# treangenlab/Seqwin

Hardware: AMD Instinct MI355X
Metric: Gbp/s minimizer-indexed (higher is better)
Workload: dtype u64

## Files before the change

seqwin_amd/csrc/device.hpp:

```cpp
#pragma once

#include <hip/hip_runtime.h>

#include <functional>
#include <memory>
#include <string>

#include "common.hpp"

namespace sw {

#define SW_HIP(expr)                                                                                   \
    do {                                                                                               \
        hipError_t _e = (expr);                                                                        \
        if (_e != hipSuccess)                                                                          \
            ::sw::raise(SW_ERR_DEVICE, "HIP error %d (%s) at %s:%d: %s", (int)_e, hipGetErrorString(_e), \
                        __FILE__, __LINE__, #expr);                                                    \
    } while (0)

__host__ __device__ inline uint64_t mix64(uint64_t x)
{
    x ^= x >> 30; x *= 0xbf58476d1ce4e5b9ULL;
    x ^= x >> 27; x *= 0x94d049bb133111ebULL;
    x ^= x >> 31;
// ... 170 lines not shown
};

namespace sw {

struct MultiGraph {
    std::vector<std::unique_ptr<sw_index>> slices;
    std::vector<uint32_t> record_offsets;
    std::string ids_blob;
    uint64_t n_assemblies = 0, total_bp = 0;
    const char *hash_route = "";
    std::string copy_route;
};
std::vector<int> devices_from_env();
void build_multi_device(const char *const *paths, size_t n_paths, uint64_t k, uint64_t w, uint64_t n_cpu, std::vector<int> devs,
                        MultiGraph &out, uint64_t chunk_bp = 0);

Plan &get_plan(sw_batch &b, uint64_t k, uint64_t w, bool *cached = nullptr);

struct SketchOut {
    DevArray<uint64_t> stage_hash;
    DevArray<uint64_t> stage_kmer;
    DevArray<uint32_t> tile_count;
    DevArray<uint64_t> tile_offset;
    uint64_t n_occ = 0;
    uint64_t launches = 0;
    uint64_t n_ovf_tiles = 0;
};
void run_sketch(const sw_batch &b, const Plan &plan, hipStream_t stream, SketchOut &out, float *sketch_ms);

void radix_sort_keys64(uint64_t *&keys, uint64_t *&alt, uint64_t n, unsigned begin_bit, unsigned end_bit, hipStream_t stream,
                       uint32_t *d_fail, bool perm_hi32 = false, unsigned long long *d_hist_given = nullptr, unsigned layout_bits = 0);
void radix_layout(unsigned bits, unsigned *digit_bits, unsigned *n_passes);
bool radix_unsort_perm(uint64_t *&keys, uint64_t *&alt, uint64_t n, unsigned low_bits, unsigned nbit, hipStream_t stream, uint32_t *d_fail);

void sort_keys64(uint64_t *&keys, uint64_t *&keys_alt, size_t n, unsigned begin_bit, unsigned end_bit, hipStream_t stream,
                 uint32_t *d_fail, bool perm_hi32 = false, unsigned long long *d_hist_given = nullptr, unsigned layout_bits = 0);
bool sort_keys64_is_own(size_t n);
void check_sort_failed(uint32_t fail_word);

struct alignas(16) OccPay {
    uint32_t low, pos, rec, idx;
};
int radix_rank_mode();
bool radix_pairs_available();
uint64_t radix_trim_state();
void radix_demote_rank();
constexpr uint32_t STAGE_WIN = 32;
constexpr uint32_t STAGE_ROW = STAGE_WIN + 9;
constexpr uint32_t STAGE_PAD = 1;
struct StageSource {
    const uint64_t *stage_hash, *stage_kmer;
    const uint32_t *tile_count;
    const uint64_t *tile_offset;
    const uint64_t *dst_off;
    uint32_t n_tiles;
    uint64_t mult;
    uint32_t *rec_out;
    const unsigned long long *chunk_dir;
    const uint64_t *rows;
};
void radix_sort_pairs32(uint32_t *&keys, uint32_t *&keys_alt, OccPay *&vals, OccPay *&vals_alt, uint64_t n, unsigned end_bit,
                        hipStream_t stream, uint32_t *d_fail, const StageSource *src = nullptr,
                        const std::function<void()> &after_first = std::function<void()>(), uint32_t *low_out = nullptr);
bool sort_pairs32(uint32_t *&keys, uint32_t *&keys_alt, OccPay *&vals, OccPay *&vals_alt, uint64_t n, unsigned end_bit,
                  hipStream_t stream, uint32_t *d_fail, uint32_t *low_out = nullptr);
struct PartState;
// ... 79 lines not shown
```

seqwin_amd/csrc/index.hip:

```cpp
#include <cstdlib>
#include <cstring>
#include <map>
#include <memory>

#include <rocprim/rocprim.hpp>

#include "device.hpp"

namespace sw {

namespace {

constexpr int TPB = 256;
inline unsigned blocks_for(uint64_t n, int per = TPB) { return (unsigned)((n + per - 1) / per); }
inline bool ranks_by_table()
{
    const char *e = SW_TEST_GETENV("SEQWIN_AMD_RANKS");
    return e && !strcmp(e, "table");
}

template <class K, class V>
void sort_pairs(K *&keys, K *&keys_alt, V *&vals, V *&vals_alt, size_t n, unsigned begin_bit, unsigned end_bit,
                hipStream_t stream)
{
// ... 2814 lines not shown
        }
    }
    DevArray<uint64_t> ukeys(m);
    DevArray<uint32_t> usum(m);
    DevArray<uint32_t> ucount(1);
    {
        auto flags = rocprim::make_transform_iterator(rocprim::make_counting_iterator<uint64_t>(0), PackedChangeAny{keys});
        const PackedPairEq eq{pshift, pmask};
        size_t tmp_bytes = 0;
        SW_HIP(rocprim::reduce_by_key(nullptr, tmp_bytes, keys, flags, m, ukeys.p, usum.p, ucount.p, rocprim::plus<uint32_t>(), eq,
                                      stream));
        DevArray<unsigned char> tmp(tmp_bytes);
        SW_HIP(rocprim::reduce_by_key(tmp.p, tmp_bytes, keys, flags, m, ukeys.p, usum.p, ucount.p, rocprim::plus<uint32_t>(), eq,
                                      stream));
        hipLaunchKernelGGL(k_drop_sentinel_run, dim3(1), dim3(1), 0, stream, ukeys.p, sentinel, ucount.p);
        SW_HIP(hipGetLastError());
        uint32_t n_edges = 0, failed = 0;
        SW_HIP(hipMemcpyAsync(&n_edges, ucount.p, 4, hipMemcpyDeviceToHost, stream));
        SW_HIP(hipMemcpyAsync(&failed, sort_fail.p, 4, hipMemcpyDeviceToHost, stream));
        SW_HIP(hipStreamSynchronize(stream));
        check_sort_failed(failed);
        ix.n_edges = n_edges;
    }
    if (ix.n_edges == 0) return;
    ix.edges.alloc(ix.n_edges);
    hipLaunchKernelGGL(k_edges_runs<false>, dim3(blocks_for(ix.n_edges)), dim3(TPB), 0, stream, ukeys.p, usum.p, pshift, pmask,
                       (uint64_t)ix.n_edges, nb, ix.nodes.p, rank_hash, ix.edges.p);
    SW_HIP(hipGetLastError());
    SW_HIP(hipStreamSynchronize(stream));
}
}

namespace {
struct WideKeys {
    unsigned lo_bits, hi_bits;
    uint64_t lo_base;
    RankHash hash;
};
void edges_from_pairs(uint64_t *keys, uint64_t *keys_alt, uint64_t m, uint64_t sentinel, unsigned nb, unsigned ab,
                      uint64_t *ck, uint32_t *ca, const unsigned long long *d_n_cand, uint64_t host_n_cand,
                      const uint64_t *rank_hash, hipStream_t stream, sw_index &ix, hipEvent_t rank_hash_ready = nullptr,
                      unsigned long long *d_hist = nullptr, const WideKeys *wide = nullptr)
{
    ix.n_edges = 0;
    if (m == 0) return;
    const unsigned key_bits = wide ? wide->lo_bits + wide->hi_bits : 2 * nb;
    DevArray<uint32_t> sort_fail(1);
    SW_HIP(hipMemsetAsync(sort_fail.p, 0, 4, stream));
    unsigned low_bits = 0, skip = 0, digit_bits = 0, n_passes = 0;
    if (sort_keys64_is_own(m)) {
        radix_layout(key_bits, &digit_bits, &n_passes);
        const unsigned hb = wide ? wide->hi_bits : nb;
        skip = hb >= digit_bits + 8 ? 1 : 0;
        if (skip && hb >= 2 * digit_bits + 8 && ix.n_nodes && m <= 4 * ix.n_nodes) skip = 2;
        if (const char *e = SW_TEST_GETENV("SEQWIN_AMD_EDGE_SKIP_PASSES")) skip = (unsigned)atoi(e);
        skip = std::min(skip, n_passes - 1);
        low_bits = skip * digit_bits;
    }
    sort_keys64(keys, keys_alt, m, low_bits, key_bits, stream, sort_fail.p, false,
                d_hist ? d_hist + ((size_t)skip << digit_bits) : nullptr, key_bits);
    RepairState rep;
    if (low_bits) enqueue_repair(EdgeKeyView{keys, low_bits}, EdgeKeyView{keys, low_bits}, ~0ull, m, nullptr, 0, rep, stream);
    DevArray<uint64_t> ukeys(m);
    DevArray<uint32_t> ucnt(m + 1), ucount(2);
    unsigned long long n_cand = host_n_cand;
    const char *rle_env = SW_AB_GETENV("SEQWIN_AMD_RLE");
    const bool own_rle = !(rle_env && !strcmp(rle_env, "rocprim"));
    bool demoted = false;
    for (int attempt = 0;; ++attempt) {
        SW_HIP(hipMemsetAsync(ucount.p + 1, 0, 4, stream));
        if (own_rle) {
            const unsigned blocks = (unsigned)((m + RLE_TILE - 1) / RLE_TILE);
            DevArray<unsigned long long> tile_state(blocks);
            DevArray<uint32_t> ticket(1);
            SW_HIP(hipMemsetAsync(tile_state.p, 0, (size_t)blocks * 8, stream));
            SW_HIP(hipMemsetAsync(ticket.p, 0, 4, stream));
            hipLaunchKernelGGL(k_rle_keys, dim3(blocks), dim3(RLE_THREADS), 0, stream, (const uint64_t *)keys, m, ukeys.p, ucnt.p, tile_state.p,
                               ticket.p, ucount.p, ucount.p + 1);
            SW_HIP(hipGetLastError());
        } else {
#ifdef SW_AB
            hipLaunchKernelGGL(k_check_ascending, dim3(blocks_for(m)), dim3(TPB), 0, stream, (const uint64_t *)keys, m, ucount.p + 1);
            size_t tmp_bytes = 0;
            SW_HIP(rocprim::run_length_encode(nullptr, tmp_bytes, keys, m, ukeys.p, ucnt.p, ucount.p, stream));
            DevArray<unsigned char> tmp(tmp_bytes);
            SW_HIP(rocprim::run_length_encode(tmp.p, tmp_bytes, keys, m, ukeys.p, ucnt.p, ucount.p, stream));
            SW_HIP(hipStreamSynchronize(stream));
#endif
        }
        hipLaunchKernelGGL(k_drop_sentinel_run, dim3(1), dim3(1), 0, stream, ukeys.p, sentinel, ucount.p);
        SW_HIP(hipGetLastError());
        uint32_t n_edges = 0, failed = 0, left = 0, descents = 0;
        SW_HIP(hipMemcpyAsync(&n_edges, ucount.p, 4, hipMemcpyDeviceToHost, stream));
        SW_HIP(hipMemcpyAsync(&descents, ucount.p + 1, 4, hipMemcpyDeviceToHost, stream));
        SW_HIP(hipMemcpyAsync(&failed, sort_fail.p, 4, hipMemcpyDeviceToHost, stream));
        if (low_bits && attempt == 0) SW_HIP(hipMemcpyAsync(&left, rep.status.p, 4, hipMemcpyDeviceToHost, stream));
        if (d_n_cand) SW_HIP(hipMemcpyAsync(&n_cand, d_n_cand, 8, hipMemcpyDeviceToHost, stream));
        SW_HIP(hipStreamSynchronize(stream));
        check_sort_failed(failed);
        if (low_bits && attempt == 0 && getenv("SEQWIN_AMD_DEBUG_EDGE_REPAIR")) {
            unsigned long long nd[2] = {0, 0};
            uint32_t st[2] = {0, 0};
// ... 1125 lines not shown
```

seqwin_amd/csrc/radix.hip:

```cpp
#include <algorithm>
#include <cstdlib>
#include <cstring>
#include <vector>
#include <map>
#include <mutex>

#include "device.hpp"

namespace sw {
namespace {

constexpr int RS_ITEMS = 16;
#ifdef SW_RS_STAMPS
__device__ unsigned long long *g_rs_stamps = nullptr;
#define RS_STAMP(i)                                                                                        \
    do {                                                                                                   \
        if (g_rs_stamps && (tile & 63u) == 0 && threadIdx.x == 0) g_rs_stamps[(size_t)(tile >> 6) * 16 + (i)] = clock64(); \
    } while (0)
#else
#define RS_STAMP(i) do { } while (0)
#endif
#ifndef RS_LOOK
#define RS_LOOK 4
#endif
// ... 33 lines not shown
{
    constexpr uint32_t RADIX = 1u << BITS;
    const unsigned p = blockIdx.x, at = begin_bit + BITS * p, sh = at - 32u, bits = min((unsigned)BITS, end_bit - at);
    const uint64_t v = threadIdx.x, block = 1ull << sh, period = block << bits;
    unsigned long long c = 0;
    if (v < (1ull << bits)) {
        const uint64_t q = n / period, r = n % period, lo = v * block;
        c = q * block + (r > lo ? (r - lo < block ? r - lo : block) : 0ull);
    }
    hist[(size_t)p * RADIX + threadIdx.x] = c;
}

constexpr uint32_t RS_CURSOR_STRIDE = 32;
template <int BITS> __global__ void k_rs_scan(unsigned long long *__restrict__ h, unsigned long long *__restrict__ cursor)
{
    constexpr uint32_t RADIX = 1u << BITS;
    __shared__ unsigned long long s[RADIX];
    const unsigned long long v = h[threadIdx.x];
    s[threadIdx.x] = v;
    __syncthreads();
    for (uint32_t d = 1; d < RADIX; d <<= 1) {
        const unsigned long long add = threadIdx.x >= d ? s[threadIdx.x - d] : 0;
        __syncthreads();
        s[threadIdx.x] += add;
        __syncthreads();
    }
    h[threadIdx.x] = s[threadIdx.x] - v;
    if (cursor) cursor[(size_t)threadIdx.x * RS_CURSOR_STRIDE] = s[threadIdx.x] - v;
}

#ifdef SW_AB
constexpr unsigned long long RS_AGG = 1ull << 62, RS_INC = 2ull << 62, RS_VAL = (1ull << 62) - 1ull;
#endif

template <int BITS>
__device__ __forceinline__ void match_digit(uint32_t d, bool live, uint32_t &mlo, uint32_t &mhi)
{
    const uint64_t lv = __ballot(live);
    mlo = (uint32_t)lv;
    mhi = (uint32_t)(lv >> 32);
#pragma unroll
    for (int b = 0; b < BITS; ++b) {
        const uint32_t sx = (uint32_t)(-(int32_t)((d >> b) & 1u));
        const uint64_t bal = __ballot(sx != 0);
        const uint32_t blo = (uint32_t)bal, bhi = (uint32_t)(bal >> 32);
        uint32_t nlo, nhi;
        asm("v_bitop3_b32 %0, %1, %2, %3 bitop3:0x90" : "=v"(nlo) : "v"(mlo), "s"(blo), "v"(sx));
        asm("v_bitop3_b32 %0, %1, %2, %3 bitop3:0x90" : "=v"(nhi) : "v"(mhi), "s"(bhi), "v"(sx));
        mlo = nlo;
        mhi = nhi;
    }
}

__global__ __launch_bounds__(1024) void k_rs_rank_selftest(uint32_t *__restrict__ mismatches)
{
    constexpr int BITS = 9;
    constexpr uint32_t RADIX = 1u << BITS, WAVES = 16;
    __shared__ uint16_t wa[WAVES][RADIX], wb[WAVES][RADIX];
    const uint32_t tid = threadIdx.x, lane = tid & 63u, wave = tid >> 6;
    for (uint32_t i = tid; i < WAVES * RADIX; i += 1024) (&wa[0][0])[i] = (&wb[0][0])[i] = 0;
    __syncthreads();
    uint32_t bad = 0;
    for (uint32_t r = 0; r < 96; ++r) {
        uint32_t x = (lane * 0x9E3779B1u) ^ ((r + 1u) * 0x85EBCA6Bu) ^ ((wave + blockIdx.x * 16u + 1u) * 0xC2B2AE35u);
        x ^= x >> 15; x *= 0x2C1B3C6Du; x ^= x >> 12;
        uint32_t d;
// ... 167 lines not shown
        goff[d] = digit_base[d] + excl - before;
    }
    __syncthreads();
#pragma unroll
    for (int i = 0; i < RS_ITEMS; ++i) {
        const uint32_t li = wave * (64 * RS_ITEMS) + i * 64 + lane;
        if (li < cnt_tile) {
            const uint32_t d = (uint32_t)(key[i] >> shift) & dmask;
            sk[lstart[d] + whist[wave][d] + rank[i]] = key[i];
        }
    }
    __syncthreads();
#pragma unroll
    for (int j = 0; j < RS_ITEMS; ++j) {
        const uint32_t t = j * THREADS + tid;
        if (t < cnt_tile) {
            const uint64_t k = sk[t];
            out[goff[(uint32_t)(k >> shift) & dmask] + t] = k;
        }
    }
}
#endif

constexpr unsigned long long RSE_VAL = (1ull << 46) - 1ull;
__device__ __forceinline__ unsigned long long rse_pack(uint32_t epoch, uint32_t flag, unsigned long long v)
{
    return ((unsigned long long)epoch << 48) | ((unsigned long long)flag << 46) | v;
}
__device__ __forceinline__ uint32_t rse_flag(unsigned long long w, uint32_t epoch)
{
    return (uint32_t)(w >> 48) == epoch ? (uint32_t)(w >> 46) & 3u : 0u;
}

template <int THREADS, int BITS, int RANK>
__global__ __launch_bounds__(THREADS) void k_rs_pass_p(const uint64_t *__restrict__ in, uint64_t *__restrict__ out, uint64_t n,
                                                       uint32_t n_tiles, unsigned shift, unsigned bits,
                                                       const unsigned long long *__restrict__ digit_base,
                                                       unsigned long long *__restrict__ state, uint32_t *__restrict__ ticket,
                                                       uint32_t *__restrict__ fail, uint32_t dbg,
                                                       unsigned long long *__restrict__ cursor, uint32_t cursor_stride,
                                                       uint32_t group_shift, uint32_t epoch)
{
    constexpr uint32_t RADIX = 1u << BITS, WAVES = THREADS / 64, TILE = THREADS * RS_ITEMS;
    static_assert(RADIX <= (uint32_t)THREADS, "one thread per digit");
    __shared__ uint64_t sk[TILE];
    __shared__ uint16_t whist[WAVES][RADIX];
    __shared__ uint32_t lstart[RADIX];
    __shared__ unsigned long long goff[RADIX];
    __shared__ uint32_t wsum[RADIX / 64];
    __shared__ uint32_t s_tile;
    const uint32_t tid = threadIdx.x, lane = tid & 63u, wave = tid >> 6;
    const uint32_t dmask = (1u << bits) - 1u;
    if (tid == 0) s_tile = atomicAdd(ticket, 1u);
    __syncthreads();
    uint32_t tile = s_tile;
    uint64_t key[RS_ITEMS];
    uint32_t rank[RS_ITEMS];
#pragma unroll
    for (int i = 0; i < RS_ITEMS; ++i) {
        const uint64_t g = (uint64_t)tile * TILE + wave * (64 * RS_ITEMS) + i * 64 + lane;
        key[i] = (tile < n_tiles && g < n) ? in[g] : ~0ull;
    }
    const uint32_t tid0 = threadIdx.x;
    uint32_t fut = 0;
    if (tid0 == 0) fut = atomicAdd(ticket, 1u);
    while (tile < n_tiles) {
        uint32_t tid = tid0;
        asm volatile("" : "+v"(tid));
        const uint32_t lane = tid & 63u, wave = tid >> 6;
        RS_STAMP(0);
        for (uint32_t i = tid; i < WAVES * RADIX / 2; i += THREADS) (reinterpret_cast<uint32_t *>(&whist[0][0]))[i] = 0;
        __syncthreads();
        const uint64_t t0 = (uint64_t)tile * TILE;
        const uint32_t cnt_tile = (uint32_t)min((uint64_t)TILE, n - t0);
        if constexpr (RANK == 1) {
#pragma unroll
            for (int i = 0; i < RS_ITEMS; ++i) {
                const uint32_t li = wave * (64 * RS_ITEMS) + i * 64 + lane;
                const uint32_t d = (uint32_t)(key[i] >> shift) & dmask;
                rank[i] = 0;
                if (li < cnt_tile) rank[i] = atomicAdd(reinterpret_cast<uint32_t *>(&whist[wave][d & ~1u]), 1u << ((d & 1u) << 4));
            }
#pragma unroll
            for (int i = 0; i < RS_ITEMS; ++i) {
                const uint32_t d = (uint32_t)(key[i] >> shift) & dmask;
                rank[i] = (rank[i] >> ((d & 1u) << 4)) & 0xFFFFu;
            }
            if ((dbg & 16u) && !cursor && wave == 0) {
#pragma unroll
                for (int i = 0; i < RS_ITEMS; ++i) {
                    const uint32_t li = i * 64 + lane;
                    const uint32_t d = li < cnt_tile ? ((uint32_t)(key[i] >> shift) & dmask) : ~lane;
                    const uint32_t od = __shfl_xor(d, 1, 64), orank = __shfl_xor(rank[i], 1, 64);
                    if (od == d) rank[i] = orank;
                }
            }
        }
#pragma unroll
        for (int i = 0; i < RS_ITEMS; ++i) {
            const uint32_t li = wave * (64 * RS_ITEMS) + i * 64 + lane;
            const bool live = li < cnt_tile;
            const uint32_t d = (uint32_t)(key[i] >> shift) & dmask;
            if constexpr (RANK == 1) {
                (void)live;
                (void)d;
            } else {
                uint32_t mlo = 1u << (lane & 31u), mhi = 0;
                if (!(dbg & 8u)) match_digit<BITS>(d, live, mlo, mhi);
                const uint32_t below = __builtin_amdgcn_mbcnt_hi(mhi, __builtin_amdgcn_mbcnt_lo(mlo, 0u));
                uint32_t prior = 0;
                if (live) prior = whist[wave][d];
                rank[i] = prior + below;
                __builtin_amdgcn_wave_barrier();
                if (live && below == 0) whist[wave][d] = (uint16_t)(prior + (uint32_t)__popc(mlo) + (uint32_t)__popc(mhi));
                __builtin_amdgcn_wave_barrier();
            }
        }
        RS_STAMP(1);
        __syncthreads();
        RS_STAMP(2);
        uint32_t total = 0, incl = 0;
        unsigned long long pre[RS_LOOK];
        unsigned long long *st = state + (size_t)tile * RADIX;
        if (tid < RADIX) {
            const uint32_t d = tid;
#pragma unroll
            for (uint32_t w = 0; w < WAVES; ++w) {
                const uint32_t c = whist[w][d];
                whist[w][d] = (uint16_t)total;
                total += c;
            }
            if (cursor) {
                const uint64_t group = group_shift < 64u ? (((uint64_t)tile * TILE) >> group_shift) : 0ull;
                pre[0] = total ? atomicAdd(&cursor[(group * RADIX + d) * cursor_stride], (unsigned long long)total) : 0ull;
            } else {
                __hip_atomic_store(&st[d], rse_pack(epoch, tile == 0 ? 2u : 1u, total), __ATOMIC_RELAXED, __HIP_MEMORY_SCOPE_AGENT);
#pragma unroll
                for (int j = 0; j < RS_LOOK; ++j)
                    pre[j] = (int64_t)tile - 1 - j >= 0
                                 ? __hip_atomic_load(&state[(size_t)(tile - 1 - j) * RADIX + d], __ATOMIC_RELAXED, __HIP_MEMORY_SCOPE_AGENT)
                                 : rse_pack(epoch, 2u, 0);
            }
            incl = total;
            for (uint32_t dd = 1; dd < 64; dd <<= 1) {
                const uint32_t up = __shfl_up(incl, dd, 64);
                if (lane >= dd) incl += up;
            }
            if (lane == 63) wsum[wave] = incl;
        }
        RS_STAMP(3);
        __syncthreads();
        uint32_t before = 0;
        if (tid < RADIX) {
            before = incl - total;
            for (uint32_t w = 0; w < wave; ++w) before += wsum[w];
            lstart[tid] = before;
        }
        if (tid == 0) s_tile = fut;
        __syncthreads();
        const uint32_t ntile = s_tile;
        auto place_and_fetch = [&]() {
#pragma unroll
            for (int i = 0; i < RS_ITEMS; ++i) {
                const uint32_t li = wave * (64 * RS_ITEMS) + i * 64 + lane;
                if (li < cnt_tile) {
                    const uint32_t d = (uint32_t)(key[i] >> shift) & dmask;
                    sk[lstart[d] + whist[wave][d] + rank[i]] = key[i];
                }
            }
#pragma unroll
            for (int i = 0; i < RS_ITEMS; ++i) {
                const uint64_t g = (uint64_t)ntile * TILE + wave * (64 * RS_ITEMS) + i * 64 + lane;
                key[i] = (ntile < n_tiles && g < n && !(dbg & 4u)) ? in[g] : (dbg & 4u ? g * 0x9E3779B97F4A7C15ull : ~0ull);
            }
            if (tid == 0) fut = atomicAdd(ticket, 1u);
        };
        const bool digit_wave = tid < RADIX;
        if (!digit_wave || cursor) place_and_fetch();
        RS_STAMP(4);
        if (tid < RADIX && cursor) {
            goff[tid] = pre[0] - before;
        } else if (tid < RADIX) {
            const uint32_t d = tid;
            unsigned long long excl = 0;
            if (tile) {
                int64_t t = (int64_t)tile - 1;
                uint32_t spins = 0;
                bool done = false;
                bool first_step = true;
#ifdef SW_RS_STAMPS
                uint32_t n_steps = 0, n_polls = 0;
#endif
                while (!done && t >= 0 && !(dbg & 1u)) {
#ifdef SW_RS_STAMPS
                    ++n_steps;
#endif
                    unsigned long long v[RS_LOOK];
#pragma unroll
                    for (int j = 0; j < RS_LOOK; ++j)
                        v[j] = first_step ? pre[j]
                               : t - j >= 0 ? __hip_atomic_load(&state[(size_t)(t - j) * RADIX + d], __ATOMIC_RELAXED, __HIP_MEMORY_SCOPE_AGENT)
                                            : rse_pack(epoch, 2u, 0);
                    first_step = false;
                    int j = 0;
#pragma unroll
                    for (; j < RS_LOOK; ++j) {
// ... 13 lines not shown
#endif
                        if (++spins > RS_SPIN_LIMIT) {
                            atomicOr(fail, 1u);
                            break;
                        }
                        __builtin_amdgcn_s_sleep(1);
                    }
                }
#ifdef SW_RS_STAMPS
                if (g_rs_stamps && (tile & 63u) == 0 && tid == 0) {
                    g_rs_stamps[(size_t)(tile >> 6) * 16 + 8] = n_steps;
                    g_rs_stamps[(size_t)(tile >> 6) * 16 + 9] = n_polls;
                    g_rs_stamps[(size_t)(tile >> 6) * 16 + 10] = (unsigned long long)((int64_t)tile - 1 - t);
                }
#endif
                __hip_atomic_store(&st[d], rse_pack(epoch, 2u, excl + total), __ATOMIC_RELAXED, __HIP_MEMORY_SCOPE_AGENT);
            }
            goff[d] = digit_base[d] + excl - before;
        }
        RS_STAMP(5);
        if (digit_wave && !cursor) place_and_fetch();
        __syncthreads();
        RS_STAMP(6);
#pragma unroll
        for (int j = 0; j < RS_ITEMS; ++j) {
            const uint32_t t = j * THREADS + tid;
            if (t < cnt_tile) {
                const uint64_t k = sk[t];
                if (!(dbg & 2u)) out[goff[(uint32_t)(k >> shift) & dmask] + t] = k;
            }
        }
        RS_STAMP(7);
        tile = ntile;
    }
}


__device__ __forceinline__ unsigned long long stage_search(const StageSource &S, uint32_t lo, uint64_t g)
{
    uint32_t hi = S.n_tiles;
    while (hi - lo > 1u) {
        const uint32_t mid = lo + ((hi - lo) >> 1);
        if (S.dst_off[mid] <= g) lo = mid; else hi = mid;
    }
    return S.tile_offset[lo] - S.dst_off[lo];
}

constexpr int RP_THREADS = 1024, RP_ITEMS = 7, RP_BITS = 8;
template <int SRC>
__global__ __launch_bounds__(RP_THREADS) void k_rs_pair_pass(const uint32_t *__restrict__ kin, const uint4 *__restrict__ pin,
                                                             uint32_t *__restrict__ kout, uint4 *__restrict__ pout, uint64_t n,
                                                             uint32_t n_tiles, unsigned shift,
                                                             const unsigned long long *__restrict__ digit_base,
                                                             unsigned long long *__restrict__ state, uint32_t epoch,
                                                             uint32_t *__restrict__ ticket, uint32_t *__restrict__ fail,
                                                             const StageSource S, uint32_t *__restrict__ lowout, uint32_t fault)
{
    constexpr bool STAGE = SRC == 1, ROWS = SRC == 2;
    constexpr uint32_t THREADS = RP_THREADS, ITEMS = RP_ITEMS, RADIX = 1u << RP_BITS, WAVES = THREADS / 64, TILE = THREADS * ITEMS;
    __shared__ uint4 sp[TILE];
    __shared__ uint32_t skey[TILE];
    __shared__ uint16_t whist[WAVES][RADIX];
    __shared__ uint32_t lstart[RADIX];
    __shared__ unsigned long long goff[RADIX];
    __shared__ uint32_t wsum[RADIX / 64];
    __shared__ uint32_t s_tile;
// ... 644 lines not shown
                           (const uint32_t *)chunk_tile.p, n, n_passes, chunk_dir.p, hist.p);
    } else {
        hipLaunchKernelGGL(k_rs_hist32, dim3((unsigned)((n + 65535) / 65536)), dim3(256), 0, stream, keys, n, n_passes, hist.p);
    }
    SW_HIP(hipGetLastError());
    StateUse su = state_buf(stream, (size_t)n_tiles * RADIX);
    StateBuf &sb = su.b;
    const StageSource none{};
    const uint32_t fault = fault_rank();
    for (unsigned p = 0; p < n_passes; ++p) {
        hipLaunchKernelGGL(k_rs_scan<RP_BITS>, dim3(1), dim3(RADIX), 0, stream, hist.p + (size_t)p * RADIX, (unsigned long long *)nullptr);
        const uint32_t epoch = next_epoch(sb, stream);
        const dim3 grid((unsigned)std::min<uint64_t>(n_tiles, (uint64_t)grid_p));
        if (p == 0 && src) {
            auto first = src->rows ? k_rs_pair_pass<2> : k_rs_pair_pass<1>;
            hipLaunchKernelGGL(first, grid, dim3(RP_THREADS), 0, stream, (const uint32_t *)nullptr, (const uint4 *)nullptr,
                               keys_alt, reinterpret_cast<uint4 *>(vals_alt), n, (uint32_t)n_tiles, 0u,
                               (const unsigned long long *)hist.p, sb.p, epoch, tickets.p, d_fail, stage,
                               n_passes == 1 ? low_out : (uint32_t *)nullptr, fault);
            SW_HIP(hipGetLastError());
            if (after_first) after_first();
        } else {
            hipLaunchKernelGGL(k_rs_pair_pass<0>, grid, dim3(RP_THREADS), 0, stream, (const uint32_t *)keys,
                               reinterpret_cast<const uint4 *>(vals), keys_alt, reinterpret_cast<uint4 *>(vals_alt), n, (uint32_t)n_tiles,
                               RP_BITS * p, (const unsigned long long *)(hist.p + (size_t)p * RADIX), sb.p, epoch, tickets.p + p, d_fail,
                               none, p + 1 == n_passes ? low_out : (uint32_t *)nullptr, fault);
            SW_HIP(hipGetLastError());
        }
        std::swap(keys, keys_alt);
        std::swap(vals, vals_alt);
    }
}

static int pick_shape(unsigned bits)
{
    const char *e = SW_TEST_GETENV("SEQWIN_AMD_RADIX_BITS");
    const bool nine = e ? atoi(e) == 9 : (bits + 8) / 9 < (bits + 7) / 8;
    const char *shape = SW_AB_GETENV("SEQWIN_AMD_RADIX_SHAPE");
    if (shape && !strcmp(shape, "1024x8")) return 2;
    if (shape && !strcmp(shape, "512x9")) return 3;
    if (shape && !strcmp(shape, "256x8")) return 4;
    return nine ? 1 : 0;
}

void radix_layout(unsigned bits, unsigned *digit_bits, unsigned *n_passes)
{
    const int sh = pick_shape(bits);
    *digit_bits = (sh == 1 || sh == 3) ? 9u : 8u;
    *n_passes = (bits + *digit_bits - 1) / *digit_bits;
}

void radix_sort_keys64(uint64_t *&keys, uint64_t *&alt, uint64_t n, unsigned begin_bit, unsigned end_bit, hipStream_t stream,
                       uint32_t *d_fail, bool perm_hi32, unsigned long long *d_hist_given, unsigned layout_bits)
{
    if (n == 0 || end_bit <= begin_bit) return;
    if (end_bit - begin_bit > 64) raise(SW_ERR_RUNTIME, "radix_sort_keys64: more than 64 key bits");
    switch (pick_shape(layout_bits ? layout_bits : end_bit - begin_bit)) {
#ifdef SW_AB
    case 2: sort_passes<1024, 8>(keys, alt, n, begin_bit, end_bit, stream, d_fail, perm_hi32, d_hist_given); break;
    case 3: sort_passes<512, 9>(keys, alt, n, begin_bit, end_bit, stream, d_fail, perm_hi32, d_hist_given); break;
    case 4: sort_passes<256, 8>(keys, alt, n, begin_bit, end_bit, stream, d_fail, perm_hi32, d_hist_given); break;
#endif
    case 1: sort_passes<1024, 9>(keys, alt, n, begin_bit, end_bit, stream, d_fail, perm_hi32, d_hist_given); break;
    default: sort_passes<512, 8>(keys, alt, n, begin_bit, end_bit, stream, d_fail, perm_hi32, d_hist_given); break;
    }
}
// ... 3 lines not shown
```

Baseline: 461.3.

## Replace full edge-key radix sort plus RLE with bucketed partition and LDS hash dedup

Measured after the change: 475.2 (median of 6 runs). 3.0% higher.

```diff
diff --git a/seqwin_amd/csrc/device.hpp b/seqwin_amd/csrc/device.hpp
--- a/seqwin_amd/csrc/device.hpp
+++ b/seqwin_amd/csrc/device.hpp
@@ -226,6 +226,10 @@
                        uint32_t *d_fail, bool perm_hi32 = false, unsigned long long *d_hist_given = nullptr, unsigned layout_bits = 0);
 void radix_layout(unsigned bits, unsigned *digit_bits, unsigned *n_passes);
 bool radix_unsort_perm(uint64_t *&keys, uint64_t *&alt, uint64_t n, unsigned low_bits, unsigned nbit, hipStream_t stream, uint32_t *d_fail);
+
+int radix_edge_buckets(uint64_t *&keys, uint64_t *&alt, uint64_t m, unsigned key_bits, uint64_t sentinel,
+                       const unsigned long long *d_hist_top, uint32_t cap, uint32_t slots, uint64_t *ukeys, uint32_t *ucnt,
+                       uint32_t *n_runs, hipStream_t stream, uint32_t *d_fail, bool debug);
 
 void sort_keys64(uint64_t *&keys, uint64_t *&keys_alt, size_t n, unsigned begin_bit, unsigned end_bit, hipStream_t stream,
                  uint32_t *d_fail, bool perm_hi32 = false, unsigned long long *d_hist_given = nullptr, unsigned layout_bits = 0);
diff --git a/seqwin_amd/csrc/index.hip b/seqwin_amd/csrc/index.hip
--- a/seqwin_amd/csrc/index.hip
+++ b/seqwin_amd/csrc/index.hip
@@ -2870,6 +2870,8 @@
 }
 
 namespace {
+constexpr uint64_t EDGE_BUCKET_MIN_KEYS = 1ull << 26;
+constexpr uint32_t EDGE_BUCKET_CAP = 1u << 20, EDGE_BUCKET_SLOTS = 4096;
 struct WideKeys {
     unsigned lo_bits, hi_bits;
     uint64_t lo_base;
@@ -2895,17 +2897,39 @@
         skip = std::min(skip, n_passes - 1);
         low_bits = skip * digit_bits;
     }
-    sort_keys64(keys, keys_alt, m, low_bits, key_bits, stream, sort_fail.p, false,
-                d_hist ? d_hist + ((size_t)skip << digit_bits) : nullptr, key_bits);
-    RepairState rep;
-    if (low_bits) enqueue_repair(EdgeKeyView{keys, low_bits}, EdgeKeyView{keys, low_bits}, ~0ull, m, nullptr, 0, rep, stream);
     DevArray<uint64_t> ukeys(m);
     DevArray<uint32_t> ucnt(m + 1), ucount(2);
     unsigned long long n_cand = host_n_cand;
     const char *rle_env = SW_AB_GETENV("SEQWIN_AMD_RLE");
     const bool own_rle = !(rle_env && !strcmp(rle_env, "rocprim"));
+    bool by_buckets = !wide && nb < 32 && own_rle && sort_keys64_is_own(m) && m >= EDGE_BUCKET_MIN_KEYS && ix.n_nodes && m > 4 * ix.n_nodes;
+    uint32_t bucket_cap = EDGE_BUCKET_CAP, bucket_slots = EDGE_BUCKET_SLOTS;
+    if (const char *e = SW_TEST_GETENV("SEQWIN_AMD_EDGE_SORT")) by_buckets = !wide && nb < 32 && own_rle && !strcmp(e, "bucket");
+    if (const char *e = SW_TEST_GETENV("SEQWIN_AMD_EDGE_BUCKET_CAP")) bucket_cap = (uint32_t)strtoul(e, nullptr, 10);
+    if (const char *e = SW_TEST_GETENV("SEQWIN_AMD_EDGE_BUCKET_SLOTS")) bucket_slots = (uint32_t)strtoul(e, nullptr, 10);
+    if (by_buckets) {
+        unsigned db = 0, np = 0;
+        radix_layout(key_bits, &db, &np);
+        uint32_t n_runs = 0;
+        by_buckets = radix_edge_buckets(keys, keys_alt, m, key_bits, sentinel, d_hist ? d_hist + ((size_t)(np - 1) << db) : nullptr, bucket_cap,
+                                        bucket_slots, ukeys.p, ucnt.p, &n_runs, stream, sort_fail.p,
+                                        getenv("SEQWIN_AMD_DEBUG_EDGE_REPAIR") != nullptr) == 0;
+        if (by_buckets) {
+            uint32_t failed = 0;
+            SW_HIP(hipMemcpyAsync(&failed, sort_fail.p, 4, hipMemcpyDeviceToHost, stream));
+            if (d_n_cand) SW_HIP(hipMemcpyAsync(&n_cand, d_n_cand, 8, hipMemcpyDeviceToHost, stream));
+            SW_HIP(hipStreamSynchronize(stream));
+            check_sort_failed(failed);
+            ix.n_edges = n_runs;
+        }
+    }
+    if (!by_buckets)
+        sort_keys64(keys, keys_alt, m, low_bits, key_bits, stream, sort_fail.p, false,
+                    d_hist ? d_hist + ((size_t)skip << digit_bits) : nullptr, key_bits);
+    RepairState rep;
+    if (low_bits && !by_buckets) enqueue_repair(EdgeKeyView{keys, low_bits}, EdgeKeyView{keys, low_bits}, ~0ull, m, nullptr, 0, rep, stream);
     bool demoted = false;
-    for (int attempt = 0;; ++attempt) {
+    for (int attempt = 0; !by_buckets; ++attempt) {
         SW_HIP(hipMemsetAsync(ucount.p + 1, 0, 4, stream));
         if (own_rle) {
             const unsigned blocks = (unsigned)((m + RLE_TILE - 1) / RLE_TILE);
diff --git a/seqwin_amd/csrc/radix.hip b/seqwin_amd/csrc/radix.hip
--- a/seqwin_amd/csrc/radix.hip
+++ b/seqwin_amd/csrc/radix.hip
@@ -89,6 +89,14 @@
 #ifdef SW_AB
 constexpr unsigned long long RS_AGG = 1ull << 62, RS_INC = 2ull << 62, RS_VAL = (1ull << 62) - 1ull;
 #endif
+
+__host__ __device__ __forceinline__ unsigned long long seg_pack(uint64_t first, uint32_t bucket, uint32_t count)
+{
+    return (unsigned long long)first << 24 | (unsigned long long)bucket << 15 | count;
+}
+__device__ __forceinline__ uint64_t seg_first(unsigned long long w) { return w >> 24; }
+__device__ __forceinline__ uint32_t seg_bucket(unsigned long long w) { return (uint32_t)(w >> 15) & 0x1FFu; }
+__device__ __forceinline__ uint32_t seg_count(unsigned long long w) { return (uint32_t)w & 0x7FFFu; }
 
 template <int BITS>
 __device__ __forceinline__ void match_digit(uint32_t d, bool live, uint32_t &mlo, uint32_t &mhi)
@@ -322,7 +330,7 @@
     return (uint32_t)(w >> 48) == epoch ? (uint32_t)(w >> 46) & 3u : 0u;
 }
 
-template <int THREADS, int BITS, int RANK>
+template <int THREADS, int BITS, int RANK, bool SEG = false>
 __global__ __launch_bounds__(THREADS) void k_rs_pass_p(const uint64_t *__restrict__ in, uint64_t *__restrict__ out, uint64_t n,
                                                        uint32_t n_tiles, unsigned shift, unsigned bits,
                                                        const unsigned long long *__restrict__ digit_base,
@@ -346,10 +354,17 @@
     uint32_t tile = s_tile;
     uint64_t key[RS_ITEMS];
     uint32_t rank[RS_ITEMS];
+    unsigned long long seg = 0, nseg = 0;
+    if constexpr (SEG) seg = tile < n_tiles ? digit_base[tile] : 0ull;
 #pragma unroll
     for (int i = 0; i < RS_ITEMS; ++i) {
-        const uint64_t g = (uint64_t)tile * TILE + wave * (64 * RS_ITEMS) + i * 64 + lane;
-        key[i] = (tile < n_tiles && g < n) ? in[g] : ~0ull;
+        const uint32_t li = wave * (64 * RS_ITEMS) + i * 64 + lane;
+        if constexpr (SEG) {
+            key[i] = li < seg_count(seg) ? in[seg_first(seg) + li] : ~0ull;
+        } else {
+            const uint64_t g = (uint64_t)tile * TILE + li;
+            key[i] = (tile < n_tiles && g < n) ? in[g] : ~0ull;
+        }
     }
     const uint32_t tid0 = threadIdx.x;
     uint32_t fut = 0;
@@ -362,7 +377,7 @@
         for (uint32_t i = tid; i < WAVES * RADIX / 2; i += THREADS) (reinterpret_cast<uint32_t *>(&whist[0][0]))[i] = 0;
         __syncthreads();
         const uint64_t t0 = (uint64_t)tile * TILE;
-        const uint32_t cnt_tile = (uint32_t)min((uint64_t)TILE, n - t0);
+        const uint32_t cnt_tile = SEG ? seg_count(seg) : (uint32_t)min((uint64_t)TILE, n - t0);
         if constexpr (RANK == 1) {
 #pragma unroll
             for (int i = 0; i < RS_ITEMS; ++i) {
@@ -421,7 +436,7 @@
                 total += c;
             }
             if (cursor) {
-                const uint64_t group = group_shift < 64u ? (((uint64_t)tile * TILE) >> group_shift) : 0ull;
+                const uint64_t group = SEG ? seg_bucket(seg) : group_shift < 64u ? (((uint64_t)tile * TILE) >> group_shift) : 0ull;
                 pre[0] = total ? atomicAdd(&cursor[(group * RADIX + d) * cursor_stride], (unsigned long long)total) : 0ull;
             } else {
                 __hip_atomic_store(&st[d], rse_pack(epoch, tile == 0 ? 2u : 1u, total), __ATOMIC_RELAXED, __HIP_MEMORY_SCOPE_AGENT);
@@ -449,6 +464,7 @@
         if (tid == 0) s_tile = fut;
         __syncthreads();
         const uint32_t ntile = s_tile;
+        if constexpr (SEG) nseg = ntile < n_tiles ? digit_base[ntile] : 0ull;
         auto place_and_fetch = [&]() {
 #pragma unroll
             for (int i = 0; i < RS_ITEMS; ++i) {
@@ -460,8 +476,13 @@
             }
 #pragma unroll
             for (int i = 0; i < RS_ITEMS; ++i) {
-                const uint64_t g = (uint64_t)ntile * TILE + wave * (64 * RS_ITEMS) + i * 64 + lane;
-                key[i] = (ntile < n_tiles && g < n && !(dbg & 4u)) ? in[g] : (dbg & 4u ? g * 0x9E3779B97F4A7C15ull : ~0ull);
+                const uint32_t li = wave * (64 * RS_ITEMS) + i * 64 + lane;
+                if constexpr (SEG) {
+                    key[i] = li < seg_count(nseg) ? in[seg_first(nseg) + li] : ~0ull;
+                } else {
+                    const uint64_t g = (uint64_t)ntile * TILE + li;
+                    key[i] = (ntile < n_tiles && g < n && !(dbg & 4u)) ? in[g] : (dbg & 4u ? g * 0x9E3779B97F4A7C15ull : ~0ull);
+                }
             }
             if (tid == 0) fut = atomicAdd(ticket, 1u);
         };
@@ -541,6 +562,7 @@
         }
         RS_STAMP(7);
         tile = ntile;
+        seg = nseg;
     }
 }
 
@@ -1251,6 +1273,378 @@
     }
 }
 
+namespace {
+constexpr uint32_t EB_RADIX = 512, EB_TABLE = EB_RADIX * EB_RADIX, EB_THREADS = 512;
+constexpr uint64_t EB_EMPTY = ~0ull;
+static_assert(EB_THREADS == EB_RADIX, "k_eb_finish: one bin per thread");
+enum : uint32_t { EB_F_OVERFLOW = 1u, EB_F_RANGE = 2u, EB_F_ORDER = 4u };
+struct EbInfo {
+    unsigned long long n_sentinels;
+    uint32_t n_tiles2, max_bucket, flags, n_runs;
+};
+
+__global__ __launch_bounds__(EB_RADIX) void k_eb_level1(const unsigned long long *__restrict__ h1, uint32_t tile_keys,
+                                                        unsigned long long *__restrict__ cursor, unsigned long long *__restrict__ segtab,
+                                                        EbInfo *__restrict__ info)
+{
+    __shared__ unsigned long long s[EB_RADIX];
+    __shared__ uint32_t st[EB_RADIX];
+    const uint32_t d = threadIdx.x;
+    const unsigned long long c = h1[d];
+    const uint32_t tiles = (uint32_t)((c + tile_keys - 1) / tile_keys);
+    s[d] = c;
+    st[d] = tiles;
+    __syncthreads();
+    for (uint32_t o = 1; o < EB_RADIX; o <<= 1) {
+        const unsigned long long a = d >= o ? s[d - o] : 0;
+        const uint32_t b = d >= o ? st[d - o] : 0;
+        __syncthreads();
+        s[d] += a;
+        st[d] += b;
+        __syncthreads();
+    }
+    const unsigned long long first = s[d] - c;
+    cursor[(size_t)d * RS_CURSOR_STRIDE] = first;
+    uint32_t w = st[d] - tiles;
+    for (uint32_t t = 0; t < tiles; ++t)
+        segtab[w + t] = seg_pack(first + (uint64_t)t * tile_keys, d, (uint32_t)min((unsigned long long)tile_keys, c - (uint64_t)t * tile_keys));
+    if (d == EB_RADIX - 1) info->n_tiles2 = st[d];
+}
+
+__global__ __launch_bounds__(1024) void k_eb_count(const uint64_t *__restrict__ in, const unsigned long long *__restrict__ segtab,
+                                                   const EbInfo *__restrict__ info, unsigned shift, uint32_t dmask, uint64_t sentinel,
+                                                   uint32_t *__restrict__ table, EbInfo *__restrict__ out)
+{
+    __shared__ uint32_t hist[EB_RADIX];
+    __shared__ uint32_t s_sent;
+    const uint32_t n_tiles = info->n_tiles2;
+    for (uint32_t w = blockIdx.x; w < n_tiles; w += gridDim.x) {
+        const unsigned long long seg = segtab[w];
+        const uint64_t first = seg_first(seg);
+        const uint32_t cnt = seg_count(seg);
+        if (threadIdx.x < EB_RADIX) hist[threadIdx.x] = 0;
+        if (threadIdx.x == 0) s_sent = 0;
+        __syncthreads();
+        uint64_t key[RS_ITEMS];
+#pragma unroll
+        for (int i = 0; i < RS_ITEMS; ++i) {
+            const uint32_t li = i * 1024 + threadIdx.x;
+            key[i] = li < cnt ? in[first + li] : EB_EMPTY;
+        }
+        uint32_t sent = 0;
+#pragma unroll
+        for (int i = 0; i < RS_ITEMS; ++i) {
+            if (key[i] == EB_EMPTY) continue;
+            if (key[i] == sentinel) ++sent;
+            atomicAdd(&hist[(uint32_t)(key[i] >> shift) & dmask], 1u);
+        }
+        if (sent) atomicAdd(&s_sent, sent);
+        __syncthreads();
+        if (threadIdx.x < EB_RADIX && hist[threadIdx.x]) atomicAdd(&table[seg_bucket(seg) * EB_RADIX + threadIdx.x], hist[threadIdx.x]);
+        if (threadIdx.x == 0 && s_sent) atomicAdd(&out->n_sentinels, (unsigned long long)s_sent);
+        __syncthreads();
+    }
+}
+
+__global__ __launch_bounds__(1024) void k_eb_scan(const uint32_t *__restrict__ cnt, const unsigned long long *__restrict__ n_sent,
+                                                  uint32_t sent_at, uint32_t *__restrict__ start, unsigned long long *__restrict__ cursor,
+                                                  uint32_t *__restrict__ max_out, uint32_t *__restrict__ total_out)
+{
+    constexpr uint32_t PER4 = EB_TABLE / 1024 / 4;
+    __shared__ uint32_t ws[16], wm[16];
+    const uint32_t tid = threadIdx.x, lane = tid & 63u, wave = tid >> 6;
+    const uint32_t sent = n_sent ? (uint32_t)*n_sent : 0u;
+    const uint4 *cnt4 = reinterpret_cast<const uint4 *>(cnt) + (size_t)tid * PER4;
+    uint32_t sum = 0, mx = 0;
+#pragma unroll 16
+    for (uint32_t j = 0; j < PER4; ++j) {
+        const uint4 c = cnt4[j];
+        mx = max(max(max(mx, c.x), max(c.y, c.z)), c.w);
+        sum += c.x + c.y + c.z + c.w;
+    }
+    if (n_sent && sent_at / (4 * PER4) == tid) {
+        mx = 0;
+        for (uint32_t j = 0; j < 4 * PER4; ++j) {
+            const uint32_t i = tid * 4 * PER4 + j, c = cnt[i];
+            mx = max(mx, c - (i == sent_at ? min(c, sent) : 0u));
+        }
+    }
+    uint32_t incl = sum;
+    for (uint32_t o = 1; o < 64; o <<= 1) {
+        const uint32_t up = __shfl_up(incl, o, 64);
+        if (lane >= o) incl += up;
+        mx = max(mx, __shfl_xor(mx, o, 64));
+    }
+    if (lane == 63) ws[wave] = incl;
+    if (lane == 0) wm[wave] = mx;
+    __syncthreads();
+    uint32_t run = incl - sum;
+    for (uint32_t w = 0; w < wave; ++w) run += ws[w];
+    uint4 *start4 = reinterpret_cast<uint4 *>(start) + (size_t)tid * PER4;
+    ulonglong2 *cur2 = reinterpret_cast<ulonglong2 *>(cursor) + (size_t)tid * PER4 * 2;
+#pragma unroll 16
+    for (uint32_t j = 0; j < PER4; ++j) {
+        const uint4 c = cnt4[j];
+        const uint4 st = make_uint4(run, run + c.x, run + c.x + c.y, run + c.x + c.y + c.z);
+        start4[j] = st;
+        if (cursor) {
+            cur2[2 * j] = make_ulonglong2(st.x, st.y);
+            cur2[2 * j + 1] = make_ulonglong2(st.z, st.w);
+        }
+        run = st.w + c.w;
+    }
+    if (tid == 1023) {
+        start[EB_TABLE] = run;
+        if (total_out) *total_out = run;
+        uint32_t m = 0;
+        for (uint32_t w = 0; w < 16; ++w) m = max(m, wm[w]);
+        if (max_out) *max_out = m;
+    }
+}
+
+__global__ __launch_bounds__(EB_THREADS) void k_eb_finish(const uint64_t *__restrict__ in, const uint32_t *__restrict__ start, uint32_t slots,
+                                                          unsigned shift1, unsigned shift2, uint32_t mask2, unsigned bin_shift,
+                                                          uint32_t bin_mask, uint64_t sentinel,
+                                                          uint64_t *__restrict__ tk, uint32_t *__restrict__ tc,
+                                                          uint32_t *__restrict__ n_distinct, uint32_t *__restrict__ flags)
+{
+    extern __shared__ __align__(16) unsigned char eb_lds[];
+    unsigned long long *hk = reinterpret_cast<unsigned long long *>(eb_lds);
+    uint32_t *hc = reinterpret_cast<uint32_t *>(hk + slots);
+    uint16_t *idx = reinterpret_cast<uint16_t *>(hc + slots);
+    __shared__ uint32_t bd[EB_RADIX + 1], bk[EB_RADIX], bcur[EB_RADIX], wsd[EB_THREADS / 64], wsk[EB_THREADS / 64];
+    __shared__ uint32_t s_over;
+    const uint32_t b = EB_TABLE - 1u - blockIdx.x, tid = threadIdx.x, lane = tid & 63u, wave = tid >> 6;
+    const uint32_t first = start[b], cnt = start[b + 1] - first;
+    if (cnt == 0) return;
+    const uint32_t mask = slots - 1u;
+    for (uint32_t s = tid; s < slots; s += EB_THREADS) {
+        hk[s] = EB_EMPTY;
+        hc[s] = 0;
+    }
+    bd[tid] = 0;
+    bk[tid] = 0;
+    if (tid == 0) s_over = 0;
+    __syncthreads();
+    uint32_t bad = 0;
+    for (uint32_t j0 = 0; j0 < cnt; j0 += 4 * EB_THREADS) {
+        if (*(volatile uint32_t *)&s_over) break;
+        uint64_t key[4];
+#pragma unroll
+        for (int i = 0; i < 4; ++i) {
+            const uint32_t j = j0 + i * EB_THREADS + tid;
+            key[i] = j < cnt ? in[(uint64_t)first + j] : sentinel;
+        }
+#pragma unroll
+        for (int i = 0; i < 4; ++i) {
+            uint64_t k = key[i];
+            bool live = k != sentinel;
+            if (live && ((uint32_t)(k >> shift1) * EB_RADIX + ((uint32_t)(k >> shift2) & mask2)) != b) {
+                bad = 1;
+                live = false;
+            }
+            uint32_t copies = 1;
+            const uint64_t any = __ballot(live);
+            if (any) {
+                const int src = __ffsll((long long)any) - 1;
+                const uint64_t k0 = (uint64_t)__shfl((unsigned long long)k, src, 64);
+                const uint64_t same = __ballot(live && k == k0);
+                if (live && k == k0) {
+                    copies = (uint32_t)__popcll(same);
+                    live = (int)lane == src;
+                }
+            }
+            if (!live) continue;
+            uint32_t h = (uint32_t)((k * 0x9E3779B97F4A7C15ull) >> 40) & mask, probes = 0;
+            for (; probes < slots; ++probes) {
+                const unsigned long long old = atomicCAS(&hk[h], EB_EMPTY, (unsigned long long)k);
+                if (old == EB_EMPTY || old == k) {
+                    atomicAdd(&hc[h], copies);
+                    break;
+                }
+                h = (h + 1u) & mask;
+            }
+            if (probes == slots) s_over = 1;
+        }
+    }
+    if (bad) atomicOr(flags, EB_F_RANGE);
+    __syncthreads();
+    if (s_over) {
+        if (tid == 0) atomicOr(flags, EB_F_OVERFLOW);
+        return;
+    }
+    for (uint32_t s = tid; s < slots; s += EB_THREADS) {
+        const uint64_t k = hk[s];
+        if (k == EB_EMPTY) continue;
+        const uint32_t bin = (uint32_t)(k >> bin_shift) & bin_mask;
+        atomicAdd(&bd[bin], 1u);
+        atomicAdd(&bk[bin], hc[s]);
+    }
+    __syncthreads();
+    {
+        const uint32_t d = bd[tid], c = bk[tid];
+        uint32_t id = d, ic = c;
+        for (uint32_t o = 1; o < 64; o <<= 1) {
+            const uint32_t ud = __shfl_up(id, o, 64), uc = __shfl_up(ic, o, 64);
+            if (lane >= o) {
+                id += ud;
+                ic += uc;
+            }
+        }
+        if (lane == 63) {
+            wsd[wave] = id;
+            wsk[wave] = ic;
+        }
+        __syncthreads();
+        uint32_t pd = id - d, pc = ic - c;
+        for (uint32_t w = 0; w < wave; ++w) {
+            pd += wsd[w];
+            pc += wsk[w];
+        }
+        bd[tid] = pd;
+        bcur[tid] = pd;
+        bk[tid] = pc;
+        if (tid == EB_THREADS - 1) bd[EB_RADIX] = pd + d;
+    }
+    __syncthreads();
+    for (uint32_t s = tid; s < slots; s += EB_THREADS) {
+        const uint64_t k = hk[s];
+        if (k == EB_EMPTY) continue;
+        idx[atomicAdd(&bcur[(uint32_t)(k >> bin_shift) & bin_mask], 1u)] = (uint16_t)s;
+    }
+    __syncthreads();
+    const uint32_t n_dist = bd[EB_RADIX];
+    if (tid == 0) n_distinct[b] = n_dist;
+    for (uint32_t j = tid; j < n_dist; j += EB_THREADS) {
+        const uint32_t s = idx[j];
+        const uint64_t k = hk[s];
+        const uint32_t bin = (uint32_t)(k >> bin_shift) & bin_mask, lo = bd[bin], hi = bd[bin + 1];
+        uint32_t less = 0, copies_less = 0;
+        for (uint32_t i = lo; i < hi; ++i) {
+            const uint32_t s2 = idx[i];
+            if (hk[s2] < k) {
+                ++less;
+                copies_less += hc[s2];
+            }
+        }
+        tk[(uint64_t)first + lo + less] = k;
+        tc[(uint64_t)first + lo + less] = first + bk[bin] + copies_less;
+    }
+}
+
+__global__ __launch_bounds__(256) void k_eb_compact(const uint64_t *__restrict__ tk, const uint32_t *__restrict__ tc,
+                                                    const uint32_t *__restrict__ start, const uint32_t *__restrict__ dstart,
+                                                    const unsigned long long *__restrict__ n_sentinels, uint64_t *__restrict__ ukeys,
+                                                    uint32_t *__restrict__ ucnt, uint32_t *__restrict__ flags)
+{
+    const uint32_t b = blockIdx.x, d0 = dstart[b], n = dstart[b + 1] - d0;
+    if (b == EB_TABLE - 1u && threadIdx.x == 0) ucnt[dstart[EB_TABLE]] = start[EB_TABLE] - (uint32_t)*n_sentinels;
+    if (n == 0) return;
+    const uint64_t first = start[b];
+    uint32_t bad = 0;
+    for (uint32_t j = threadIdx.x; j < n; j += 256) {
+        const uint64_t k = tk[first + j];
+        const uint32_t c = tc[first + j];
+        if (j + 1 < n && (tk[first + j + 1] <= k || tc[first + j + 1] <= c)) bad = 1;
+        if (c < first || c >= start[b + 1]) bad = 1;
+        ukeys[d0 + j] = k;
+        ucnt[d0 + j] = c;
+    }
+    if (bad) atomicOr(flags, EB_F_ORDER);
+}
+}
+
+int radix_edge_buckets(uint64_t *&keys, uint64_t *&alt, uint64_t m, unsigned key_bits, uint64_t sentinel,
+                       const unsigned long long *d_hist_top, uint32_t cap, uint32_t slots, uint64_t *ukeys, uint32_t *ucnt,
+                       uint32_t *n_runs, hipStream_t stream, uint32_t *d_fail, bool debug)
+{
+    constexpr int THREADS = 1024, BITS = 9;
+    constexpr uint32_t TILE = THREADS * RS_ITEMS;
+    unsigned digit_bits = 0, n_passes = 0;
+    radix_layout(key_bits, &digit_bits, &n_passes);
+    if (n_passes < 2 || m >= (1ull << 32) - 1 || slots < 64 || slots > 8192 || (slots & (slots - 1))) return 1;
+    const unsigned shift1 = (n_passes - 1) * digit_bits, bits1 = key_bits - shift1;
+    const unsigned bits2 = std::min<unsigned>(BITS, shift1), shift2 = shift1 - bits2;
+    const unsigned bin_bits = std::min<unsigned>(BITS, shift2), bin_shift = shift2 - bin_bits;
+    const uint64_t n_tiles = (m + TILE - 1) / TILE, max_tiles2 = n_tiles + EB_RADIX;
+    int dev = 0, per_cu = 0;
+    SW_HIP(hipGetDevice(&dev));
+    hipDeviceProp_t prop;
+    SW_HIP(hipGetDeviceProperties(&prop, dev));
+    SW_HIP(hipOccupancyMaxActiveBlocksPerMultiprocessor(&per_cu, k_rs_pass_p<THREADS, BITS, 0>, THREADS, 0));
+    const unsigned cus = (unsigned)std::max(1, prop.multiProcessorCount);
+    const unsigned grid = (unsigned)std::min<uint64_t>(n_tiles, (uint64_t)std::max(1, per_cu) * cus);
+
+    DevArray<unsigned long long> h1(EB_RADIX), cur1((size_t)EB_RADIX * RS_CURSOR_STRIDE), cur2(EB_TABLE), segtab(max_tiles2);
+    DevArray<uint32_t> table(EB_TABLE), start(EB_TABLE + 1), tickets(2), flags(1);
+    DevArray<EbInfo> info(1);
+    SW_HIP(hipMemsetAsync(h1.p, 0, h1.bytes(), stream));
+    SW_HIP(hipMemsetAsync(table.p, 0, table.bytes(), stream));
+    SW_HIP(hipMemsetAsync(tickets.p, 0, 8, stream));
+    SW_HIP(hipMemsetAsync(flags.p, 0, 4, stream));
+    SW_HIP(hipMemsetAsync(info.p, 0, sizeof(EbInfo), stream));
+    if (d_hist_top)
+        SW_HIP(hipMemcpyAsync(h1.p, d_hist_top, (size_t)8 << digit_bits, hipMemcpyDeviceToDevice, stream));
+    else
+        hipLaunchKernelGGL(k_rs_hist<BITS>, dim3((unsigned)((m + 32767) / 32768)), dim3(256), 0, stream, (const uint64_t *)keys, m, shift1,
+                           key_bits, 1u, h1.p);
+    hipLaunchKernelGGL(k_eb_level1, dim3(1), dim3(EB_RADIX), 0, stream, (const unsigned long long *)h1.p, TILE, cur1.p, segtab.p, info.p);
+    auto pass1 = ballot_forced() ? k_rs_pass_p<THREADS, BITS, 0> : k_rs_pass_p<THREADS, BITS, 1>;
+    hipLaunchKernelGGL(pass1, dim3(grid), dim3(THREADS), 0, stream, (const uint64_t *)keys, alt, m, (uint32_t)n_tiles, shift1, bits1,
+                       (const unsigned long long *)nullptr, (unsigned long long *)nullptr, tickets.p, d_fail, 0u, cur1.p, RS_CURSOR_STRIDE,
+                       64u, 0u);
+    std::swap(keys, alt);
+    hipLaunchKernelGGL(k_eb_count, dim3((unsigned)std::min<uint64_t>(max_tiles2, (uint64_t)8 * cus)), dim3(1024), 0, stream,
+                       (const uint64_t *)keys, (const unsigned long long *)segtab.p, (const EbInfo *)info.p, shift2, (1u << bits2) - 1u,
+                       sentinel, table.p, info.p);
+    const uint32_t sent_at = (uint32_t)(sentinel >> shift1) * EB_RADIX + ((uint32_t)(sentinel >> shift2) & ((1u << bits2) - 1u));
+    hipLaunchKernelGGL(k_eb_scan, dim3(1), dim3(1024), 0, stream, (const uint32_t *)table.p, (const unsigned long long *)&info.p->n_sentinels,
+                       sent_at, start.p, cur2.p, &info.p->max_bucket, (uint32_t *)nullptr);
+    SW_HIP(hipGetLastError());
+    EbInfo hi;
+    SW_HIP(hipMemcpyAsync(&hi, info.p, sizeof hi, hipMemcpyDeviceToHost, stream));
+    SW_HIP(hipStreamSynchronize(stream));
+    if (debug)
+        fprintf(stderr, "[edge buckets] %llu keys, %llu sentinels, digits %u+%u+%u of %u bits, largest sub-bucket %u (capacity %u, %u slots)%s\n",
+                (unsigned long long)m, hi.n_sentinels, bits1, bits2, bin_bits, key_bits, hi.max_bucket, cap, slots,
+                hi.max_bucket > cap ? ": radix passes instead" : "");
+    if (hi.max_bucket > cap) return 1;
+    auto pass2 = ballot_forced() ? k_rs_pass_p<THREADS, BITS, 0, true> : k_rs_pass_p<THREADS, BITS, 1, true>;
+    hipLaunchKernelGGL(pass2, dim3(std::max(1u, std::min(hi.n_tiles2, (uint32_t)(std::max(1, per_cu) * cus)))), dim3(THREADS), 0, stream,
+                       (const uint64_t *)keys, alt, m, hi.n_tiles2, shift2, bits2, (const unsigned long long *)segtab.p,
+                       (unsigned long long *)nullptr, tickets.p + 1, d_fail, 0u, cur2.p, 1u, 64u, 0u);
+    std::swap(keys, alt);
+    DevArray<uint32_t> tc(m), n_distinct(EB_TABLE), dstart(EB_TABLE + 1);
+    SW_HIP(hipMemsetAsync(n_distinct.p, 0, n_distinct.bytes(), stream));
+    uint64_t *tk = alt;
+    const size_t lds = (size_t)slots * 14;
+    static std::mutex &mu = *new std::mutex;
+    {
+        std::lock_guard<std::mutex> lock(mu);
+        SW_HIP(hipFuncSetAttribute(reinterpret_cast<const void *>(k_eb_finish), hipFuncAttributeMaxDynamicSharedMemorySize, (int)lds));
+    }
+    hipLaunchKernelGGL(k_eb_finish, dim3(EB_TABLE), dim3(EB_THREADS), lds, stream, (const uint64_t *)keys, (const uint32_t *)start.p, slots,
+                       shift1, shift2, (1u << bits2) - 1u, bin_shift, (1u << bin_bits) - 1u, sentinel, tk, tc.p, n_distinct.p, flags.p);
+    hipLaunchKernelGGL(k_eb_scan, dim3(1), dim3(1024), 0, stream, (const uint32_t *)n_distinct.p, (const unsigned long long *)nullptr, 0u,
+                       dstart.p, (unsigned long long *)nullptr, (uint32_t *)nullptr, &info.p->n_runs);
+    hipLaunchKernelGGL(k_eb_compact, dim3(EB_TABLE), dim3(256), 0, stream, (const uint64_t *)tk, (const uint32_t *)tc.p,
+                       (const uint32_t *)start.p, (const uint32_t *)dstart.p, (const unsigned long long *)&info.p->n_sentinels, ukeys, ucnt,
+                       flags.p);
+    SW_HIP(hipGetLastError());
+    uint32_t hf = 0;
+    SW_HIP(hipMemcpyAsync(&hi, info.p, sizeof hi, hipMemcpyDeviceToHost, stream));
+    SW_HIP(hipMemcpyAsync(&hf, flags.p, 4, hipMemcpyDeviceToHost, stream));
+    SW_HIP(hipStreamSynchronize(stream));
+    if (hf & (EB_F_RANGE | EB_F_ORDER))
+        raise(SW_ERR_RUNTIME, "internal error: the edge buckets are out of order (%s)", hf & EB_F_RANGE ? "a key outside its bucket" : "run starts descend");
+    if (hf & EB_F_OVERFLOW) {
+        if (debug) fprintf(stderr, "[edge buckets] a sub-bucket holds more than %u distinct keys: radix passes instead\n", slots);
+        return 1;
+    }
+    *n_runs = hi.n_runs;
+    return 0;
+}
+
 static int pick_shape(unsigned bits)
 {
     const char *e = SW_TEST_GETENV("SEQWIN_AMD_RADIX_BITS");
```
